# hellosunking/Microcket

Hardware: NVIDIA B200
Metric: valid pairs/sec (SAM->dedup->binned) (higher is better)
Workload: dtype u8

## Files before the change

microcket_b200/csrc/pairs.cu:

```cuda
#include <algorithm>
#include <vector>
#include "mk_common.cuh"
#include "radix_sort.cuh"
#include "pairs_ws.h"

struct K64 {
    typedef u64 Key;
    static constexpr int ITEMS = 16;
    static constexpr int MIN_BLOCKS = 1;
    static constexpr bool HAS_VAL = false;
    struct Bufs { u64 *k[2]; u32 *v[2]; };
    __device__ static __forceinline__ u32 digit(const u64 &k, int byte) { return (u32)(k >> (8 * byte)) & 255u; }
    __device__ static __forceinline__ u64 load_key(const Bufs &b, int which, u64 i) { return b.k[which][i]; }
    __device__ static __forceinline__ void store_key(const Bufs &b, int which, u64 i, const u64 &k) { b.k[which][i] = k; }
};

#define UQ_T 256
#define UQ_ITEMS 8

__global__ void __launch_bounds__(256) k_mark_first(const u64 *k0, const u64 *k1, const u32 *v0, const u32 *v1, const RadixPlan *plan,
                                                    u64 n, u8 *keep, unsigned long long *n_unique) {
    const u64 *k = plan->final_buf ? k1 : k0;
    const u32 *v = plan->final_buf ? v1 : v0;
    u32 local = 0;
    for (u64 i = (u64)blockIdx.x * blockDim.x + threadIdx.x; i < n; i += (u64)gridDim.x * blockDim.x) {
        bool first = i == 0 || k[i] != k[i - 1];
        keep[plan->n_exec ? v[i] : (u32)i] = first ? 1 : 0;
        local += first;
    }
    local = __reduce_add_sync(0xffffffffu, local);
    if ((threadIdx.x & 31) == 0 && local) atomicAdd(n_unique, (unsigned long long)local);
}

__device__ __forceinline__ bool pair_key_differs(const uint4 &a, const uint4 &b) {
    return a.x != b.x || a.y != b.y || a.z != b.z || ((a.w ^ b.w) & 0xFFFF00FFu) != 0;
}

__global__ void __launch_bounds__(UQ_T) k_unique_rec16(const uint4 *b0, const uint4 *b1, const RadixPlan *plan, u64 n,
                                                       uint4 *o0, uint4 *o1, u64 *desc, unsigned long long *n_out, u32 *ticket) {
    __shared__ u32 s_scan[UQ_T / 32 + 1];
    __shared__ u64 s_base;
    __shared__ u32 s_tile;
    const uint4 *in = plan->final_buf ? b1 : b0;
    uint4 *out = plan->final_buf ? o0 : o1;
    const int tid = threadIdx.x, lane = tid & 31, wid = tid >> 5;
    const int n_tiles = (int)((n + UQ_T * UQ_ITEMS - 1) / (UQ_T * UQ_ITEMS));
    while (true) {
        if (tid == 0) s_tile = atomicAdd(ticket, 1u);
        __syncthreads();
        const int tile = (int)s_tile;
        if (tile >= n_tiles) break;
        const u64 base = (u64)tile * UQ_T * UQ_ITEMS + (u64)tid * UQ_ITEMS;
        uint4 r[UQ_ITEMS]; u32 f = 0, cnt = 0;
        uint4 prev = base > 0 && base <= n ? in[base - 1] : make_uint4(0, 0, 0, 0);
#pragma unroll
        for (int k = 0; k < UQ_ITEMS; ++k) {
            if (base + k < n) {
                r[k] = in[base + k];
                bool first = (base + k == 0) || pair_key_differs(r[k], prev);
                prev = r[k];
                if (first) { f |= 1u << k; ++cnt; }
            }
        }
        u32 tot;
        u32 ex = block_excl_scan<UQ_T>(cnt, s_scan, &tot);
        if (wid == 0) {
            u64 b = lookback_exclusive(desc, tile, 0, tot, lane);
            if (lane == 0) { s_base = b; if (tile == n_tiles - 1) *n_out = b + tot; }
        }
        __syncthreads();
        u64 o = s_base + ex;
// ... 44 lines not shown
}

__global__ void k_rle_trim(const u64 *key, const u32 *pos, unsigned long long *counters , u64 n, u64 cap) {
    const u64 runs = counters[0];
    counters[2] = n;
    if (runs && runs <= cap && key[runs - 1] == 0xFFFFFFFFFFFFFFFFull) { counters[0] = runs - 1; counters[2] = pos[runs - 1]; }
}
__global__ void k_rle_finish(const u64 *key, const u32 *pos, const unsigned long long *nnz_p, u64 n_unused, u64 cap,
                             u32 *bin1, u32 *bin2, u32 *cnt) {
    const u64 n = nnz_p[2];
    const u64 nnz = *nnz_p < cap ? *nnz_p : cap;
    for (u64 i = (u64)blockIdx.x * blockDim.x + threadIdx.x; i < nnz; i += (u64)gridDim.x * blockDim.x) {
        u64 k = key[i];
        bin1[i] = (u32)(k >> 32); bin2[i] = (u32)k;
        u32 nxt = (i + 1 < *nnz_p && i + 1 < cap) ? pos[i + 1] : (u32)n;
        if (i + 1 < *nnz_p && i + 1 >= cap) nxt = pos[i] + 1;
        cnt[i] = nxt - pos[i];
    }
}

#define BIN_BAD_KEY 0xFFFFFFFFFFFFFFFFull
__global__ void k_bin_keys(const mk_pair *p, u64 n, const u32 *chr_off , const u32 *chr_len , u32 n_ids,
                           u32 res, u64 *key, unsigned long long *bad) {
    u32 nbad = 0;
    for (u64 i = (u64)blockIdx.x * blockDim.x + threadIdx.x; i < n; i += (u64)gridDim.x * blockDim.x) {
        const uint4 r = ((const uint4 *)p)[i];
        const u32 pos1 = r.x, pos2 = r.y, c1 = r.z & 0xFFFFu, c2 = r.z >> 16;
        u64 k = BIN_BAD_KEY;
        if (c1 < n_ids && c2 < n_ids && pos1 <= chr_len[c1] && pos2 <= chr_len[c2]) {
            u32 a = chr_off[c1] + pos1 / res, b = chr_off[c2] + pos2 / res;
            if (a > b) { u32 t = a; a = b; b = t; }
            k = ((u64)a << 32) | b;
        }
        nbad += k == BIN_BAD_KEY;
        key[i] = k;
    }
    nbad = __reduce_add_sync(0xffffffffu, nbad);
    if ((threadIdx.x & 31) == 0 && nbad) atomicAdd(bad, (unsigned long long)nbad);
}

extern "C" int mk_pairs_ws_create(int device, size_t max_pairs, mk_pairs_ws **out) {
    if (!out || max_pairs == 0) { mk_set_error("mk_pairs_ws_create: bad argument"); return MK_ERR_ARG; }
    int ndev = 0;
    if (cudaGetDeviceCount(&ndev) != cudaSuccess || ndev == 0) { mk_set_error("no CUDA device: microcket_b200 has no CPU fallback"); return MK_ERR_CUDA; }
    MK_CUDA(cudaSetDevice(device));
    mk_pairs_ws *w = new mk_pairs_ws();
    w->device = device; w->sms = mk_sm_count(device); w->max_pairs = max_pairs;
    int rc = w->rws.alloc(max_pairs);
    if (rc == MK_OK) rc = w->alt.alloc(max_pairs * 16);
    if (rc == MK_OK) rc = w->keys2.alloc(max_pairs * 8);
    if (rc == MK_OK) rc = w->heads_key.alloc(max_pairs * 8);
    if (rc == MK_OK) rc = w->heads_pos.alloc(max_pairs * 4);
    if (rc == MK_OK) rc = w->desc.alloc((max_pairs / (UQ_T * UQ_ITEMS) + 4) * 8 + 2048);
    if (rc == MK_OK) rc = w->counter.alloc(64);
    if (rc == MK_OK) rc = w->chr_off.alloc(65536 * 8 + 16384 * 8);
    if (rc == MK_OK && cudaMemset(w->chr_off.p, 0, w->chr_off.n) != cudaSuccess) rc = MK_ERR_CUDA;
    if (rc != MK_OK) { delete w; return rc; }
    *out = w;
    return MK_OK;
}
extern "C" void mk_pairs_ws_destroy(mk_pairs_ws *w) { if (w) { cudaSetDevice(w->device); delete w; } }
extern "C" uint64_t mk_pairs_launch_count(mk_pairs_ws *w) { return w ? w->launches : 0; }
extern "C" uint64_t mk_pairs_dropped(mk_pairs_ws *w) { return w ? w->dropped : 0; }

static int lookback_grid(const void *kernel, int threads, int sms) {
    int occ = 1;
    cudaOccupancyMaxActiveBlocksPerMultiprocessor(&occ, kernel, threads, 0);
    return sms * std::max(1, std::min(occ, 4));
}

extern "C" int mk_pairs_dedup_device(mk_pairs_ws *w, mk_pair *d_pairs, size_t n, size_t *n_kept, void *stream) {
    if (!w || !n_kept) { mk_set_error("mk_pairs_dedup_device: bad argument"); return MK_ERR_ARG; }
    if (n > w->max_pairs) { mk_set_error("mk_pairs_dedup_device: workspace holds %zu pairs, got %zu", w->max_pairs, n); return MK_ERR_CAPACITY; }
    MK_CUDA(cudaSetDevice(w->device));
    cudaStream_t s = (cudaStream_t)stream;
    if (n == 0) { *n_kept = 0; return MK_OK; }
    RadixSchedule sch; sch.n_pass = 15;
    const int order[15] = {12, 4, 5, 6, 7, 10, 11, 0, 1, 2, 3, 8, 9, 14, 15};
    for (int i = 0; i < 15; ++i) sch.byte_of[i] = order[i];
    Rec16::Bufs b; b.k[0] = (uint4 *)d_pairs; b.k[1] = w->alt.as<uint4>(); b.v[0] = b.v[1] = nullptr;
    MK_TRY(radix_sort<Rec16>(b, n, sch, w->rws, 0, w->sms, s, &w->launches));
    const int n_tiles = (int)((n + UQ_T * UQ_ITEMS - 1) / (UQ_T * UQ_ITEMS));
    MK_CUDA(cudaMemsetAsync(w->desc.p, 0, (size_t)(n_tiles + 1) * 8, s));
    MK_CUDA(cudaMemsetAsync(w->counter.p, 0, 64, s));
    k_unique_rec16<<<lookback_grid((const void *)k_unique_rec16, UQ_T, w->sms), UQ_T, 0, s>>>(
        b.k[0], b.k[1], w->rws.plan.as<RadixPlan>(), n, b.k[0], b.k[1], w->desc.as<u64>(), w->counter.as<unsigned long long>(),
        (u32 *)(w->counter.as<unsigned long long>() + 4));
    w->launches += 1;
    struct { unsigned long long kept; } hc;
    u32 final_buf = 0;
    MK_CUDA(cudaMemcpyAsync(&hc, w->counter.p, 8, cudaMemcpyDeviceToHost, s));
    MK_CUDA(cudaMemcpyAsync(&final_buf, (char *)w->rws.plan.p + offsetof(RadixPlan, final_buf), 4, cudaMemcpyDeviceToHost, s));
    MK_CUDA(cudaStreamSynchronize(s));
    if (final_buf == 0) MK_CUDA(cudaMemcpyAsync(d_pairs, w->alt.p, (size_t)hc.kept * 16, cudaMemcpyDeviceToDevice, s));
    *n_kept = (size_t)hc.kept;
    MK_CUDA(cudaStreamSynchronize(s));
    return MK_OK;
}

extern "C" int mk_pairs_bin_device(mk_pairs_ws *w, const mk_pair *d_pairs, size_t n, const uint32_t *chrom_len, int n_chrom,
                                   const uint16_t *chrom_id_map, int n_map, uint32_t res, uint32_t *d_bin1, uint32_t *d_bin2,
                                   uint32_t *d_cnt, size_t cap, size_t *nnz, void *stream) {
    if (!w || !nnz || !chrom_len || n_chrom <= 0 || res == 0) { mk_set_error("mk_pairs_bin_device: bad argument"); return MK_ERR_ARG; }
    if (n > w->max_pairs) { mk_set_error("mk_pairs_bin_device: workspace holds %zu pairs, got %zu", w->max_pairs, n); return MK_ERR_CAPACITY; }
    MK_CUDA(cudaSetDevice(w->device));
    cudaStream_t s = (cudaStream_t)stream;
    if (n == 0) { *nnz = 0; return MK_OK; }
    std::vector<u64> off(n_chrom + 1, 0);
    for (int c = 0; c < n_chrom; ++c) off[c + 1] = off[c] + chrom_len[c] / res + 1;
    if (off[n_chrom] >= (1ull << 32)) { mk_set_error("mk_pairs_bin_device: more than 2^32 bins"); return MK_ERR_CAPACITY; }
    const int n_ids = chrom_id_map ? n_map : n_chrom;
    if (n_ids > 65536) { mk_set_error("mk_pairs_bin_device: too many chromosome ids"); return MK_ERR_ARG; }
    std::vector<u32> by_id(2 * (size_t)n_ids);
    for (int i = 0; i < n_ids; ++i) {
        int c = chrom_id_map ? chrom_id_map[i] : i;
        if (c < 0 || c >= n_chrom) { mk_set_error("mk_pairs_bin_device: chromosome map entry %d out of range", i); return MK_ERR_ARG; }
        by_id[i] = (u32)off[c]; by_id[n_ids + i] = chrom_len[c];
    }
    MK_CUDA(cudaMemcpyAsync(w->chr_off.p, by_id.data(), by_id.size() * 4, cudaMemcpyHostToDevice, s));
    MK_CUDA(cudaMemsetAsync(w->counter.p, 0, 64, s));
// ... 99 lines not shown
        u32 peers = __match_any_sync(0xffffffffu, d);
        if (i < n && lane == __ffs(peers) - 1) atomicAdd(&s_c[d], (u32)__popc(peers));
    }
    __syncthreads();
    if (threadIdx.x < world && s_c[threadIdx.x]) atomicAdd(&counts[threadIdx.x], (unsigned long long)s_c[threadIdx.x]);
}

__global__ void __launch_bounds__(256) k_owner_scatter(const mk_pair *p, u64 n, u32 world, u32 res, unsigned long long *cursor ,
                                                       mk_pair *out) {
    const int lane = threadIdx.x & 31;
    const u64 n_round = (n + 31) & ~(u64)31;
    for (u64 i = (u64)blockIdx.x * blockDim.x + threadIdx.x; i < n_round; i += (u64)gridDim.x * blockDim.x) {
        u32 d = 0xFFFFu + lane; uint4 r = make_uint4(0, 0, 0, 0);
        if (i < n) { r = ((const uint4 *)p)[i]; d = mk_owner_hash(r.z & 0xFFFFu, r.z >> 16, r.x / res) % world; }
        u32 peers = __match_any_sync(0xffffffffu, d);
        int leader = __ffs(peers) - 1;
        unsigned long long base = 0;
        if (i < n && lane == leader) base = atomicAdd(&cursor[d], (unsigned long long)__popc(peers));
        base = __shfl_sync(0xffffffffu, base, leader);
        if (i < n) ((uint4 *)out)[base + __popc(peers & ((1u << lane) - 1u))] = r;
    }
}

__global__ void k_owner_prefix(unsigned long long *dc, u32 world) {
    unsigned long long run = 0;
    for (u32 r = 0; r < world; ++r) { dc[64 + r] = run; run += dc[r]; }
}

extern "C" int mk_pairs_partition_device(mk_pairs_ws *w, const mk_pair *d_pairs, size_t n, int world, uint32_t res, mk_pair *d_out,
                                         uint64_t *counts, void *stream) {
    if (!w || !counts || world < 1 || world > 64 || res == 0 || (n && (!d_pairs || !d_out))) { mk_set_error("mk_pairs_partition_device: bad argument"); return MK_ERR_ARG; }
    if (n > w->max_pairs) { mk_set_error("mk_pairs_partition_device: workspace holds %zu pairs, got %zu", w->max_pairs, n); return MK_ERR_CAPACITY; }
    MK_CUDA(cudaSetDevice(w->device));
    cudaStream_t s = (cudaStream_t)stream;
    unsigned long long *dc = (unsigned long long *)w->desc.p;
    MK_CUDA(cudaMemsetAsync(dc, 0, 128 * 8, s));
    if (n) {
        k_owner_count<<<w->sms * 8, 256, 0, s>>>(d_pairs, n, (u32)world, res, dc);
        k_owner_prefix<<<1, 1, 0, s>>>(dc, (u32)world);
    }
    unsigned long long h[64];
    MK_CUDA(cudaMemcpyAsync(h, dc, (size_t)world * 8, cudaMemcpyDeviceToHost, s));
    if (n) k_owner_scatter<<<w->sms * 8, 256, 0, s>>>(d_pairs, n, (u32)world, res, dc + 64, d_out);
    w->launches += n ? 3 : 0;
    MK_CUDA(cudaStreamSynchronize(s));
    for (int r = 0; r < world; ++r) counts[r] = h[r];
    return MK_OK;
}

extern "C" uint32_t mk_pairs_owner(uint32_t chr1, uint32_t chr2, uint32_t pos1, uint32_t res, uint32_t world) {
    return mk_owner_hash(chr1, chr2, pos1 / res) % world;
}

struct PackCfg { u32 res, nb, nr, nl, total_bits, n_dec, n_ids, max_lane; };

__device__ __forceinline__ void put_bits(u64 &lo, u64 &hi, u64 v, u32 width) {
    hi = width >= 64 ? lo << (width - 64) : (width ? (hi << width) | (lo >> (64 - width)) : hi);
    lo = width >= 64 ? 0 : lo << width;
    lo |= v;
}
__device__ __forceinline__ u64 take_bits(u64 &lo, u64 &hi, u32 width) {
    const u64 v = width >= 64 ? lo : (lo & ((1ull << width) - 1));
    lo = width >= 64 ? hi : (width ? (lo >> width) | (hi << (64 - width)) : lo);
    hi = width >= 64 ? 0 : hi >> width;
    return v;
}

__global__ void __launch_bounds__(256) k_pack_keys(const mk_pair *p, u64 n, const u32 *off_by_id, const u32 *len_by_id, PackCfg c, uint4 *key,
                                                   unsigned long long *bad, RadixSchedule sch, RadixPlan *plan) {
    extern __shared__ u32 s_hist[];
    for (int i = threadIdx.x; i < sch.n_pass * 256; i += 256) s_hist[i] = 0;
    __syncthreads();
    const int lane_id = threadIdx.x & 31;
    u32 nbad = 0;
    const u64 n_round = (n + 31) & ~(u64)31;
    for (u64 i = (u64)blockIdx.x * blockDim.x + threadIdx.x; i < n_round; i += (u64)gridDim.x * blockDim.x) {
        const bool valid = i < n;
        uint4 k = make_uint4(0xFFFFFFFFu, 0xFFFFFFFFu, 0xFFFFFFFFu, (u32)i);
        if (valid) {
            const uint4 r = ((const uint4 *)p)[i];
            u32 pos1 = r.x, pos2 = r.y; const u32 c1 = r.z & 0xFFFFu, c2 = r.z >> 16;
            u32 st = r.w & 3u; const u32 lane = r.w >> 16;
            bool ok = c1 < c.n_ids && c2 < c.n_ids && lane <= c.max_lane;
            if (ok) {
                const u32 q1 = pos1 / c.res, q2 = pos2 / c.res;
                ok = pos1 <= len_by_id[c1] && pos2 <= len_by_id[c2];
                if (ok) {
                    u32 a = off_by_id[c1] + q1, b = off_by_id[c2] + q2;
                    u32 r1 = pos1 - q1 * c.res, r2 = pos2 - q2 * c.res;
                    u32 sw = 0;
                    if (a > b) { u32 t = a; a = b; b = t; t = r1; r1 = r2; r2 = t; st = ((st & 1u) << 1) | (st >> 1); sw = 1; }
                    u64 lo = 0, hi = 0;
                    put_bits(lo, hi, a, c.nb); put_bits(lo, hi, b, c.nb); put_bits(lo, hi, lane, c.nl);
                    put_bits(lo, hi, r1, c.nr); put_bits(lo, hi, r2, c.nr); put_bits(lo, hi, sw, 1); put_bits(lo, hi, st, 2);
                    k.x = (u32)lo; k.y = (u32)(lo >> 32); k.z = (u32)hi;
                }
            }
            nbad += !ok;
            key[i] = k;
        }
        radix_hist_add<Rec16>(s_hist, sch, k, valid, lane_id);
    }
    nbad = __reduce_add_sync(0xffffffffu, nbad);
    if ((threadIdx.x & 31) == 0 && nbad) atomicAdd(bad, (unsigned long long)nbad);
    __syncthreads();
    radix_hist_flush(s_hist, sch.n_pass, plan);
}

__device__ __forceinline__ u32 chrom_of_bin(u32 bin, u32 hint, const PackCfg &c, const u32 *dec_off) {
    if (dec_off[hint] <= bin && (hint + 1 == c.n_dec || bin < dec_off[hint + 1])) return hint;
    u32 l = 0, h = c.n_dec - 1;
    while (l < h) { const u32 m = (l + h + 1) >> 1; if (dec_off[m] <= bin) l = m; else h = m - 1; }
    return l;
}
__device__ __forceinline__ mk_pair unpack_key(uint4 k, const PackCfg &c, const u32 *dec_off, const u16 *dec_id, u32 &hint) {
    u64 lo = (u64)k.x | ((u64)k.y << 32), hi = (u64)k.z;
    u32 st = (u32)take_bits(lo, hi, 2); const u32 sw = (u32)take_bits(lo, hi, 1);
    u32 r2 = (u32)take_bits(lo, hi, c.nr), r1 = (u32)take_bits(lo, hi, c.nr);
    const u32 lane = (u32)take_bits(lo, hi, c.nl);
    u32 b = (u32)take_bits(lo, hi, c.nb), a = (u32)take_bits(lo, hi, c.nb);
    u32 ka = chrom_of_bin(a, hint, c, dec_off);
    u32 kb = chrom_of_bin(b, ka, c, dec_off);
    hint = ka;
    if (sw) { u32 t = a; a = b; b = t; t = r1; r1 = r2; r2 = t; t = ka; ka = kb; kb = t; st = ((st & 1u) << 1) | (st >> 1); }
    mk_pair o;
    o.pos1 = (a - dec_off[ka]) * c.res + r1; o.pos2 = (b - dec_off[kb]) * c.res + r2;
    o.chr1 = dec_id[ka]; o.chr2 = dec_id[kb]; o.strands = (u8)st; o.lane = (u16)lane;
    if (o.chr1 != o.chr2) o.cls = 0;
    else { const u32 d = o.pos2 - o.pos1; o.cls = d >= 10000u ? 1 : (d >= 1000u ? 2 : 3); }
    return o;
}

__global__ void __launch_bounds__(UQ_T) k_uniq_cells(const uint4 *b0, const uint4 *b1, const RadixPlan *plan, u64 n, PackCfg c,
                                                     const u32 *dec_off, const u16 *dec_id, mk_pair *out0, mk_pair *out1,
                                                     u32 *cell_b1, u32 *cell_b2, u32 *cell_first, u64 cell_cap, u8 *keep, u32 *kept_idx,
                                                     u64 *desc, unsigned long long *counters , u32 *ticket) {
    __shared__ u32 s_w[2][UQ_T / 32];
    __shared__ u64 s_base;
    __shared__ u32 s_tile;
    const uint4 *in = plan->final_buf ? b1 : b0;
    mk_pair *out = plan->final_buf ? out0 : out1;
    const int tid = threadIdx.x, lane = tid & 31, wid = tid >> 5;
    const int n_tiles = (int)((n + UQ_T * UQ_ITEMS - 1) / (UQ_T * UQ_ITEMS));
    const u32 cell_shift = c.total_bits - 2 * c.nb;
    while (true) {
        if (tid == 0) s_tile = atomicAdd(ticket, 1u);
        __syncthreads();
        const int tile = (int)s_tile;
        if (tile >= n_tiles) break;
        const u64 base = (u64)tile * UQ_T * UQ_ITEMS + (u64)tid * UQ_ITEMS;
        uint4 r[UQ_ITEMS]; u32 fk = 0, fc = 0, nk = 0, nc = 0;
        uint4 prev = base > 0 && base <= n ? in[base - 1] : make_uint4(0, 0, 0, 0);
#pragma unroll
        for (int k = 0; k < UQ_ITEMS; ++k) {
            if (base + k < n) {
                r[k] = in[base + k];
                const bool first = base + k == 0;
                const bool dk = first || r[k].x != prev.x || r[k].y != prev.y || r[k].z != prev.z;
                bool dc = first;
                if (!first && dk) {
                    u64 lo = (u64)r[k].x | ((u64)r[k].y << 32), hi = (u64)r[k].z;
                    u64 plo = (u64)prev.x | ((u64)prev.y << 32), phi = (u64)prev.z;
                    take_bits(lo, hi, cell_shift); take_bits(plo, phi, cell_shift);
                    dc = lo != plo || hi != phi;
                }
                prev = r[k];
                if (dk) { fk |= 1u << k; ++nk; }
                if (dc) { fc |= 1u << k; ++nc; }
            }
        }
        const u32 ik = warp_incl_scan(nk, lane), ic = warp_incl_scan(nc, lane);
        if (lane == 31) { s_w[0][wid] = ik; s_w[1][wid] = ic; }
        __syncthreads();
        u32 bk = 0, bc = 0, tk = 0, tc = 0;
#pragma unroll
        for (int w = 0; w < UQ_T / 32; ++w) { const u32 x = s_w[0][w], y = s_w[1][w]; tk += x; tc += y; if (w < wid) { bk += x; bc += y; } }
        if (wid == 0) {
            const u64 agg = (u64)tk | ((u64)tc << 31);
            const u64 b = lookback_exclusive(desc, tile, 0, agg, lane);
            if (lane == 0) { s_base = b; if (tile == n_tiles - 1) { counters[0] = (b & 0x7FFFFFFFu) + tk; counters[1] = (b >> 31) + tc; } }
        }
        __syncthreads();
        u64 ok = (s_base & 0x7FFFFFFFu) + bk + ik - nk, oc = (s_base >> 31) + bc + ic - nc;
        u32 hint = 0;
#pragma unroll
        for (int k = 0; k < UQ_ITEMS; ++k) {
            if (fc & (1u << k)) {
                if (oc < cell_cap) {
                    u64 lo = (u64)r[k].x | ((u64)r[k].y << 32), hi = (u64)r[k].z;
                    take_bits(lo, hi, cell_shift);
                    const u32 bb = (u32)take_bits(lo, hi, c.nb), aa = (u32)take_bits(lo, hi, c.nb);
                    cell_b1[oc] = aa; cell_b2[oc] = bb; cell_first[oc] = (u32)ok;
                }
                ++oc;
            }
            if (fk & (1u << k)) {
                out[ok] = unpack_key(r[k], c, dec_off, dec_id, hint);
                if (keep) keep[r[k].w] = 1;
                if (kept_idx) kept_idx[ok] = r[k].w;
                ++ok;
            }
        }
        __syncthreads();
    }
}

__global__ void k_uniq_trim(const uint4 *b0, const uint4 *b1, const RadixPlan *plan, u64 n, u8 *keep, unsigned long long *counters) {
    const uint4 *in = plan->final_buf ? b1 : b0;
    if (!counters[3]) return;
    const u64 first_bad = n - counters[3];
    const uint4 k = in[first_bad];
    if (k.x == 0xFFFFFFFFu && k.y == 0xFFFFFFFFu && k.z == 0xFFFFFFFFu) {
        counters[0] -= 1; counters[1] -= 1;
        if (keep) keep[k.w] = 0;
    }
}

__global__ void k_cell_counts(const u32 *cell_first, const unsigned long long *counters, u64 cap, u32 *cnt) {
    const u64 kept = counters[0], cells = counters[1] < cap ? counters[1] : cap;
    for (u64 i = (u64)blockIdx.x * blockDim.x + threadIdx.x; i < cells; i += (u64)gridDim.x * blockDim.x)
        cnt[i] = (i + 1 < counters[1] && i + 1 < cap ? cell_first[i + 1] : (u32)kept) - cell_first[i];
}

__global__ void k_copy_if_alt(const RadixPlan *plan, u32 keys_in_home_when, const uint4 *alt, uint4 *home, const unsigned long long *counters) {
    if (plan->final_buf != keys_in_home_when) return;
    const u64 n = counters[0];
    for (u64 i = (u64)blockIdx.x * blockDim.x + threadIdx.x; i < n; i += (u64)gridDim.x * blockDim.x) home[i] = alt[i];
}

static u32 bits_for(u64 max_value) { u32 b = 1; while (b < 64 && (max_value >> b)) ++b; return b; }

extern "C" int mk_pairs_dedup_bin_indexed_device(mk_pairs_ws *w, mk_pair *d_pairs, size_t n, const uint32_t *chrom_len, int n_chrom,
                                                 const uint16_t *chrom_id_map, int n_map, uint32_t res, uint16_t max_lane,
                                                 uint32_t *d_bin1, uint32_t *d_bin2, uint32_t *d_cnt, size_t cap,
                                                 uint8_t *d_keep, uint32_t *d_kept_idx, size_t *n_kept, size_t *nnz, void *stream) {
    if (!w || !n_kept || !nnz || !chrom_len || n_chrom <= 0 || res == 0 || !d_bin1 || !d_bin2 || !d_cnt) { mk_set_error("mk_pairs_dedup_bin_device: bad argument"); return MK_ERR_ARG; }
    if (n > w->max_pairs) { mk_set_error("mk_pairs_dedup_bin_device: workspace holds %zu pairs, got %zu", w->max_pairs, n); return MK_ERR_CAPACITY; }
    MK_CUDA(cudaSetDevice(w->device));
    cudaStream_t s = (cudaStream_t)stream;
    *n_kept = 0; *nnz = 0; w->dropped = 0;
    if (n == 0) return MK_OK;
    std::vector<u64> off(n_chrom + 1, 0);
    for (int c = 0; c < n_chrom; ++c) off[c + 1] = off[c] + chrom_len[c] / res + 1;
    if (off[n_chrom] >= (1ull << 32)) { mk_set_error("mk_pairs_dedup_bin_device: more than 2^32 bins"); return MK_ERR_CAPACITY; }
    const int n_ids = chrom_id_map ? n_map : n_chrom;
    if (n_ids > 16384 || n_chrom > 16384) { mk_set_error("mk_pairs_dedup_bin_device: too many chromosomes"); return MK_ERR_ARG; }
    std::vector<u32> tab(3 * 16384 + 8192, 0);
    u32 *by_id = tab.data(), *nb_id = by_id + 16384, *dec_off = nb_id + 16384; u16 *dec_id = (u16 *)(dec_off + 16384);
    for (int c = 0; c < n_chrom; ++c) { dec_off[c] = (u32)off[c]; dec_id[c] = 0xFFFF; }
    for (int i = 0; i < n_ids; ++i) {
        int c = chrom_id_map ? chrom_id_map[i] : i;
        if (c < 0 || c >= n_chrom) { mk_set_error("mk_pairs_dedup_bin_device: chromosome map entry %d out of range", i); return MK_ERR_ARG; }
        by_id[i] = (u32)off[c]; nb_id[i] = chrom_len[c];
        if (dec_id[c] == 0xFFFF) dec_id[c] = (u16)i;
    }
    PackCfg pc; pc.res = res; pc.nb = bits_for(off[n_chrom]) ;
    pc.nr = bits_for(res - 1); pc.nl = max_lane ? bits_for(max_lane) : 0;
    pc.total_bits = 2 * pc.nb + 2 * pc.nr + pc.nl + 3; pc.n_dec = (u32)n_chrom; pc.n_ids = (u32)n_ids; pc.max_lane = max_lane;
    if (pc.total_bits > 96) { mk_set_error("mk_pairs_dedup_bin_device: key needs %u bits, 96 available", pc.total_bits); return MK_ERR_CAPACITY; }
    u32 *d_by_id = w->chr_off.as<u32>(), *d_nb_id = d_by_id + 16384, *d_dec_off = d_nb_id + 16384; u16 *d_dec_id = (u16 *)(d_dec_off + 16384);
    MK_CUDA(cudaMemcpyAsync(d_by_id, tab.data(), tab.size() * 4, cudaMemcpyHostToDevice, s));
    MK_CUDA(cudaMemsetAsync(w->counter.p, 0, 64, s));
    unsigned long long *cnt = w->counter.as<unsigned long long>();
    if (d_keep) MK_CUDA(cudaMemsetAsync(d_keep, 0, n, s));
    RadixSchedule sch; sch.n_pass = (int)((pc.total_bits + 7) / 8);
    for (int i = 0; i < sch.n_pass; ++i) sch.byte_of[i] = i;
    const bool in_place = (sch.n_pass & 1) != 0;
    uint4 *k0 = in_place ? (uint4 *)d_pairs : w->alt.as<uint4>(), *k1 = in_place ? w->alt.as<uint4>() : (uint4 *)d_pairs;
    MK_CUDA(cudaMemsetAsync(w->rws.plan.p, 0, sizeof(RadixPlan), s));
    k_pack_keys<<<w->sms * 8, 256, sch.n_pass * 256 * 4, s>>>(d_pairs, n, d_by_id, d_nb_id, pc, k0, cnt + 3, sch, w->rws.plan.as<RadixPlan>());
    w->launches += 1;
    Rec16::Bufs b; b.k[0] = k0; b.k[1] = k1; b.v[0] = b.v[1] = nullptr;
    MK_TRY(radix_sort<Rec16>(b, n, sch, w->rws, 0, w->sms, s, &w->launches, true));
    const int n_tiles = (int)((n + UQ_T * UQ_ITEMS - 1) / (UQ_T * UQ_ITEMS));
    MK_CUDA(cudaMemsetAsync(w->desc.p, 0, (size_t)(n_tiles + 1) * 8, s));
    const RadixPlan *plan = w->rws.plan.as<RadixPlan>();
    k_uniq_cells<<<lookback_grid((const void *)k_uniq_cells, UQ_T, w->sms), UQ_T, 0, s>>>(
        k0, k1, plan, n, pc, d_dec_off, d_dec_id, (mk_pair *)k0, (mk_pair *)k1,
        d_bin1, d_bin2, w->heads_pos.as<u32>(), cap, d_keep, d_kept_idx, w->desc.as<u64>(), cnt, (u32 *)(cnt + 4));
    k_uniq_trim<<<1, 1, 0, s>>>(k0, k1, plan, n, d_keep, cnt);
    k_cell_counts<<<w->sms * 4, 256, 0, s>>>(w->heads_pos.as<u32>(), cnt, cap, d_cnt);
    k_copy_if_alt<<<w->sms * 4, 256, 0, s>>>(plan, in_place ? 0u : 1u, w->alt.as<uint4>(), (uint4 *)d_pairs, cnt);
    w->launches += 4;
    unsigned long long h[4];
    MK_CUDA(cudaMemcpyAsync(h, cnt, 32, cudaMemcpyDeviceToHost, s));
    MK_CUDA(cudaStreamSynchronize(s));
    *n_kept = (size_t)h[0]; *nnz = (size_t)h[1]; w->dropped = h[3];
    if (h[1] > cap) { mk_set_error("mk_pairs_dedup_bin_device: %llu non-zero cells, output capacity %zu", h[1], cap); return MK_ERR_CAPACITY; }
    return MK_OK;
}

extern "C" int mk_pairs_dedup_bin_device(mk_pairs_ws *w, mk_pair *d_pairs, size_t n, const uint32_t *chrom_len, int n_chrom,
                                         const uint16_t *chrom_id_map, int n_map, uint32_t res, uint16_t max_lane,
                                         uint32_t *d_bin1, uint32_t *d_bin2, uint32_t *d_cnt, size_t cap,
                                         size_t *n_kept, size_t *nnz, void *stream) {
    return mk_pairs_dedup_bin_indexed_device(w, d_pairs, n, chrom_len, n_chrom, chrom_id_map, n_map, res, max_lane, d_bin1, d_bin2, d_cnt, cap,
                                             nullptr, nullptr, n_kept, nnz, stream);
}
```

microcket_b200/csrc/pairs_ws.h:

```cpp
#pragma once
#include "mk_common.cuh"
#include "radix_sort.cuh"

struct mk_pairs_ws {
    int device = 0, sms = 148;
    size_t max_pairs = 0;
    RadixWs rws;
    DevBuf alt;
    DevBuf keys2;
    DevBuf heads_key, heads_pos;
    DevBuf desc, counter, chr_off;
    DevBuf h_pairs, h_b1, h_b2, h_c;
    DevBuf sort2;
    DevBuf tile_sum, tile_off; size_t text_tiles = 0;
    DevBuf names, nl;
    u64 launches = 0;
    u64 dropped = 0;
    int text_scratch(size_t n_tiles) {
        if (n_tiles <= text_tiles) return MK_OK;
        MK_TRY(tile_sum.alloc(n_tiles * 4)); MK_TRY(tile_off.alloc(n_tiles * 8));
        text_tiles = n_tiles;
        return MK_OK;
    }
};
```

Measured before the change: 1.873 billion.

## Stage uniq tile loads and pair outputs through padded shared memory for coalescing

Loads each tile of sorted 16-byte keys into padded shared memory with a coalesced strided pattern, instead of each thread reading eight consecutive records. Unpacked mk_pair outputs are compacted into the same shared buffer and then written to global memory coalesced as uint4. The aim is to replace uncoalesced per-thread global loads and scattered stores with contiguous transactions. In exchange it adds about 66KB of shared memory per block, which may reduce occupancy, plus two extra block barriers, and it relies on mk_pair fitting in 16 bytes.

Measured after the change: 1.889 billion, median of 6. About the same (+0.9%).

```diff
diff --git a/microcket_b200/csrc/pairs.cu b/microcket_b200/csrc/pairs.cu
--- a/microcket_b200/csrc/pairs.cu
+++ b/microcket_b200/csrc/pairs.cu
@@ -465,6 +465,7 @@
     return o;
 }
 
+#define UQ_PAD(i) ((i) + (i) / UQ_ITEMS)
 __global__ void __launch_bounds__(UQ_T) k_uniq_cells(const uint4 *b0, const uint4 *b1, const RadixPlan *plan, u64 n, PackCfg c,
                                                      const u32 *dec_off, const u16 *dec_id, mk_pair *out0, mk_pair *out1,
                                                      u32 *cell_b1, u32 *cell_b2, u32 *cell_first, u64 cell_cap, u8 *keep, u32 *kept_idx,
@@ -472,8 +473,9 @@
     __shared__ u32 s_w[2][UQ_T / 32];
     __shared__ u64 s_base;
     __shared__ u32 s_tile;
+    __shared__ uint4 s_rec[UQ_PAD(UQ_T * UQ_ITEMS)];
     const uint4 *in = plan->final_buf ? b1 : b0;
-    mk_pair *out = plan->final_buf ? out0 : out1;
+    uint4 *out = (uint4 *)(plan->final_buf ? out0 : out1);
     const int tid = threadIdx.x, lane = tid & 31, wid = tid >> 5;
     const int n_tiles = (int)((n + UQ_T * UQ_ITEMS - 1) / (UQ_T * UQ_ITEMS));
     const u32 cell_shift = c.total_bits - 2 * c.nb;
@@ -482,13 +484,20 @@
         __syncthreads();
         const int tile = (int)s_tile;
         if (tile >= n_tiles) break;
-        const u64 base = (u64)tile * UQ_T * UQ_ITEMS + (u64)tid * UQ_ITEMS;
+        const u64 tile_base = (u64)tile * UQ_T * UQ_ITEMS, base = tile_base + (u64)tid * UQ_ITEMS;
+        const u32 n_tile = (u32)min((u64)UQ_T * UQ_ITEMS, n - tile_base);
+#pragma unroll
+        for (int k = 0; k < UQ_ITEMS; ++k) {
+            const u32 i = k * UQ_T + tid;
+            if (i < n_tile) s_rec[UQ_PAD(i)] = in[tile_base + i];
+        }
+        __syncthreads();
         uint4 r[UQ_ITEMS]; u32 fk = 0, fc = 0, nk = 0, nc = 0;
-        uint4 prev = base > 0 && base <= n ? in[base - 1] : make_uint4(0, 0, 0, 0);
+        uint4 prev = base > 0 && base <= n ? (tid ? s_rec[UQ_PAD(tid * UQ_ITEMS - 1)] : in[base - 1]) : make_uint4(0, 0, 0, 0);
 #pragma unroll
         for (int k = 0; k < UQ_ITEMS; ++k) {
             if (base + k < n) {
-                r[k] = in[base + k];
+                r[k] = s_rec[UQ_PAD(tid * UQ_ITEMS + k)];
                 const bool first = base + k == 0;
                 const bool dk = first || r[k].x != prev.x || r[k].y != prev.y || r[k].z != prev.z;
                 bool dc = first;
@@ -515,7 +524,9 @@
             if (lane == 0) { s_base = b; if (tile == n_tiles - 1) { counters[0] = (b & 0x7FFFFFFFu) + tk; counters[1] = (b >> 31) + tc; } }
         }
         __syncthreads();
-        u64 ok = (s_base & 0x7FFFFFFFu) + bk + ik - nk, oc = (s_base >> 31) + bc + ic - nc;
+        const u64 tile_k = s_base & 0x7FFFFFFFu;
+        u32 lk = bk + ik - nk;
+        u64 oc = (s_base >> 31) + bc + ic - nc;
         u32 hint = 0;
 #pragma unroll
         for (int k = 0; k < UQ_ITEMS; ++k) {
@@ -524,17 +535,19 @@
                     u64 lo = (u64)r[k].x | ((u64)r[k].y << 32), hi = (u64)r[k].z;
                     take_bits(lo, hi, cell_shift);
                     const u32 bb = (u32)take_bits(lo, hi, c.nb), aa = (u32)take_bits(lo, hi, c.nb);
-                    cell_b1[oc] = aa; cell_b2[oc] = bb; cell_first[oc] = (u32)ok;
+                    cell_b1[oc] = aa; cell_b2[oc] = bb; cell_first[oc] = (u32)(tile_k + lk);
                 }
                 ++oc;
             }
             if (fk & (1u << k)) {
-                out[ok] = unpack_key(r[k], c, dec_off, dec_id, hint);
+                *(mk_pair *)&s_rec[UQ_PAD(lk)] = unpack_key(r[k], c, dec_off, dec_id, hint);
                 if (keep) keep[r[k].w] = 1;
-                if (kept_idx) kept_idx[ok] = r[k].w;
-                ++ok;
+                if (kept_idx) kept_idx[tile_k + lk] = r[k].w;
+                ++lk;
             }
         }
+        __syncthreads();
+        for (u32 i = tid; i < tk; i += UQ_T) out[tile_k + i] = s_rec[UQ_PAD(i)];
         __syncthreads();
     }
 }
```

## Replace full LSD radix sort with top-byte sort plus in-shared-memory segment sort

Applied to the files above, without the earlier changes.

The dedup/bin path now radix-sorts only the top three key bytes globally. Windows of 2048 records are then finished with an in-shared-memory LSD sort over only the low bytes that actually vary. Prefix groups that overflow a window are gathered, fully sorted by a separate global radix sort, and scattered back. The single lookback unique kernel becomes per-tile count, scan and emit kernels. This cuts global sort passes, at the cost of a host sync mid-pipeline, extra launches, and complex boundary logic.

New measurement: 1.873 billion before, 1.938 billion after, median of 6. 3.5% higher.

```diff
diff --git a/microcket_b200/csrc/pairs.cu b/microcket_b200/csrc/pairs.cu
--- a/microcket_b200/csrc/pairs.cu
+++ b/microcket_b200/csrc/pairs.cu
@@ -17,6 +17,10 @@
 
 #define UQ_T 256
 #define UQ_ITEMS 8
+#define DB_T 2048
+#define DB_THREADS 512
+#define DB_ITEMS 8
+#define DB_WARPS (DB_THREADS / 32)
 
 __global__ void __launch_bounds__(256) k_mark_first(const u64 *k0, const u64 *k1, const u32 *v0, const u32 *v1, const RadixPlan *plan,
                                                     u64 n, u8 *keep, unsigned long long *n_unique) {
@@ -167,6 +171,7 @@
     if (rc == MK_OK) rc = w->heads_key.alloc(max_pairs * 8);
     if (rc == MK_OK) rc = w->heads_pos.alloc(max_pairs * 4);
     if (rc == MK_OK) rc = w->desc.alloc((max_pairs / (UQ_T * UQ_ITEMS) + 4) * 8 + 2048);
+    if (rc == MK_OK) rc = w->seg.alloc((max_pairs / DB_T + 2) * 5 * 4);
     if (rc == MK_OK) rc = w->counter.alloc(64);
     if (rc == MK_OK) rc = w->chr_off.alloc(65536 * 8 + 16384 * 8);
     if (rc == MK_OK && cudaMemset(w->chr_off.p, 0, w->chr_off.n) != cudaSuccess) rc = MK_ERR_CUDA;
@@ -178,9 +183,9 @@
 extern "C" uint64_t mk_pairs_launch_count(mk_pairs_ws *w) { return w ? w->launches : 0; }
 extern "C" uint64_t mk_pairs_dropped(mk_pairs_ws *w) { return w ? w->dropped : 0; }
 
-static int lookback_grid(const void *kernel, int threads, int sms) {
+static int lookback_grid(const void *kernel, int threads, int sms, size_t smem = 0) {
     int occ = 1;
-    cudaOccupancyMaxActiveBlocksPerMultiprocessor(&occ, kernel, threads, 0);
+    cudaOccupancyMaxActiveBlocksPerMultiprocessor(&occ, kernel, threads, smem);
     return sms * std::max(1, std::min(occ, 4));
 }
 
@@ -386,7 +391,7 @@
     return mk_owner_hash(chr1, chr2, pos1 / res) % world;
 }
 
-struct PackCfg { u32 res, nb, nr, nl, total_bits, n_dec, n_ids, max_lane; };
+struct PackCfg { u32 res, nb, nr, nl, total_bits, n_dec, n_ids, max_lane, pshift , pbits ; };
 
 __device__ __forceinline__ void put_bits(u64 &lo, u64 &hi, u64 v, u32 width) {
     hi = width >= 64 ? lo << (width - 64) : (width ? (hi << width) | (lo >> (64 - width)) : hi);
@@ -465,77 +470,234 @@
     return o;
 }
 
-__global__ void __launch_bounds__(UQ_T) k_uniq_cells(const uint4 *b0, const uint4 *b1, const RadixPlan *plan, u64 n, PackCfg c,
-                                                     const u32 *dec_off, const u16 *dec_id, mk_pair *out0, mk_pair *out1,
-                                                     u32 *cell_b1, u32 *cell_b2, u32 *cell_first, u64 cell_cap, u8 *keep, u32 *kept_idx,
-                                                     u64 *desc, unsigned long long *counters , u32 *ticket) {
-    __shared__ u32 s_w[2][UQ_T / 32];
-    __shared__ u64 s_base;
-    __shared__ u32 s_tile;
+__device__ __forceinline__ u32 key_prefix(const uint4 &r, const PackCfg &c) {
+    u64 lo = (u64)r.x | ((u64)r.y << 32), hi = (u64)r.z;
+    take_bits(lo, hi, c.pshift);
+    return (u32)lo & ((1u << c.pbits) - 1u);
+}
+__device__ u64 prefix_bound(const uint4 *in, const PackCfg &c, u64 lo, u64 hi, u32 p, bool upper) {
+    while (lo < hi) {
+        const u64 m = (lo + hi) >> 1;
+        const u32 q = key_prefix(in[m], c);
+        if (q < p || (upper && q == p)) lo = m + 1; else hi = m;
+    }
+    return lo;
+}
+
+__global__ void k_over_find(const uint4 *b0, const uint4 *b1, const RadixPlan *plan, u64 n, PackCfg c, u32 n_win, u32 *seg_start, u32 *seg_len) {
+    const uint4 *in = plan->final_buf ? b1 : b0;
+    for (u32 t = blockIdx.x * blockDim.x + threadIdx.x; t < n_win; t += gridDim.x * blockDim.x) {
+        const u64 a = (u64)t * DB_T, e = a + DB_T < n ? a + DB_T : n;
+        u64 start = 0, len = 0;
+        if (t >= 1) {
+            const u32 p = key_prefix(in[a - 1], c);
+            if (key_prefix(in[e - 1], c) == p && !(t >= 2 && key_prefix(in[a - DB_T - 1], c) == p)) {
+                start = prefix_bound(in, c, 0, a - 1, p, false);
+                len = prefix_bound(in, c, e, n, p, true) - start;
+            }
+        }
+        seg_start[t] = (u32)start; seg_len[t] = (u32)len;
+    }
+}
+
+__global__ void __launch_bounds__(1024) k_scan_windows(const u32 *cnt, u32 n_win, u32 *off, unsigned long long *total) {
+    __shared__ u32 s_scan[1024 / 32 + 1];
+    const u32 per = (n_win + 1023) / 1024, b = threadIdx.x * per, e = b + per < n_win ? b + per : n_win;
+    u32 sum = 0;
+    for (u32 t = b; t < e; ++t) sum += cnt[t];
+    u32 tot;
+    u32 run = block_excl_scan<1024>(sum, s_scan, &tot);
+    for (u32 t = b; t < e; ++t) { off[t] = run; run += cnt[t]; }
+    if (threadIdx.x == 0) { off[n_win] = tot; *total = tot; }
+}
+
+__device__ __forceinline__ u32 over_src(u32 j, const u32 *off, const u32 *seg_start, u32 n_win) {
+    u32 lo = 0, hi = n_win;
+    while (lo < hi) { const u32 m = (lo + hi + 1) >> 1; if (off[m] <= j) lo = m; else hi = m - 1; }
+    return seg_start[lo] + (j - off[lo]);
+}
+__global__ void k_over_gather(const uint4 *data, uint4 *scr, u32 m, const u32 *off, const u32 *seg_start, u32 n_win) {
+    for (u32 j = blockIdx.x * blockDim.x + threadIdx.x; j < m; j += gridDim.x * blockDim.x) scr[j] = data[over_src(j, off, seg_start, n_win)];
+}
+__global__ void k_over_scatter(uint4 *data, const uint4 *s0, const uint4 *s1, const RadixPlan *plan, u32 m, const u32 *off, const u32 *seg_start, u32 n_win) {
+    const uint4 *scr = plan->final_buf ? s1 : s0;
+    for (u32 j = blockIdx.x * blockDim.x + threadIdx.x; j < m; j += gridDim.x * blockDim.x) data[over_src(j, off, seg_start, n_win)] = scr[j];
+}
+
+__device__ __forceinline__ void seg_flags(const uint4 r, const uint4 p, bool first, u32 cell_shift, bool &dk, bool &dc) {
+    dk = first || r.x != p.x || r.y != p.y || r.z != p.z;
+    dc = first;
+    if (!first && dk) {
+        u64 rl = (u64)r.x | ((u64)r.y << 32), rh = (u64)r.z, pl = (u64)p.x | ((u64)p.y << 32), ph = (u64)p.z;
+        take_bits(rl, rh, cell_shift); take_bits(pl, ph, cell_shift);
+        dc = rl != pl || rh != ph;
+    }
+}
+
+struct SegSmem {
+    uint4 rec[2 * DB_T];
+    u32 wc[DB_WARPS * 256];
+    u32 dig[256];
+    u32 scan[DB_WARPS + 1];
+    u32 vary[3];
+    u32 lo, hi, nk, nc;
+};
+
+__device__ __forceinline__ void seg_sort_pass(SegSmem &s, u32 lo, u32 L, u32 byte, int tid, int lane, int wid) {
+    for (int i = tid; i < DB_WARPS * 256; i += DB_THREADS) s.wc[i] = 0;
+    __syncthreads();
+    uint4 r[DB_ITEMS]; u32 rank[DB_ITEMS / 2] = {};
+    u32 *wc = s.wc + wid * 256;
+    const u32 wbase = (u32)wid * 32 * DB_ITEMS;
+#pragma unroll
+    for (int j = 0; j < DB_ITEMS; ++j) {
+        if (wbase + j * 32 >= L) break;
+        const u32 q = wbase + j * 32 + lane;
+        u32 d = 255u;
+        if (q < L) { r[j] = s.rec[lo + q]; d = Rec16::digit(r[j], byte); }
+        u32 peers = 0xffffffffu;
+#pragma unroll
+        for (int bit = 0; bit < 8; ++bit) { const bool on = (d >> bit) & 1u; const u32 bl = __ballot_sync(0xffffffffu, on); peers &= on ? bl : ~bl; }
+        const int leader = __ffs(peers) - 1;
+        u32 old = 0;
+        if (lane == leader) { old = wc[d]; wc[d] = old + (u32)__popc(peers); }
+        old = __shfl_sync(0xffffffffu, old, leader);
+        rank[j / 2] |= (old + (u32)__popc(peers & ((1u << lane) - 1u))) << (16 * (j & 1));
+        __syncwarp();
+    }
+    __syncthreads();
+    u32 cnt = 0;
+    if (tid < 256) {
+#pragma unroll
+        for (int w = 0; w < DB_WARPS; ++w) { const u32 x = s.wc[w * 256 + tid]; s.wc[w * 256 + tid] = cnt; cnt += x; }
+    }
+    u32 tot;
+    const u32 ex = block_excl_scan<DB_THREADS>(cnt, s.scan, &tot);
+    if (tid < 256) s.dig[tid] = ex;
+    __syncthreads();
+#pragma unroll
+    for (int j = 0; j < DB_ITEMS; ++j) {
+        const u32 q = wbase + j * 32 + lane;
+        if (q < L) { const u32 d = Rec16::digit(r[j], byte); s.rec[lo + s.dig[d] + wc[d] + ((rank[j / 2] >> (16 * (j & 1))) & 0xFFFFu)] = r[j]; }
+    }
+    __syncthreads();
+}
+
+__global__ void __launch_bounds__(DB_THREADS, 2) k_seg_sort(uint4 *b0, uint4 *b1, const RadixPlan *plan, u64 n, PackCfg c,
+                                                            u32 *tile_lo, u32 *kept_cnt, u32 *cell_cnt) {
+    extern __shared__ __align__(16) unsigned char s_raw[];
+    SegSmem &s = *(SegSmem *)s_raw;
+    uint4 *in = plan->final_buf ? b1 : b0;
+    const int tid = threadIdx.x, lane = tid & 31, wid = tid >> 5;
+    const u32 n_win = (u32)((n + DB_T - 1) / DB_T), n_pass = (c.pshift + c.pbits) / 8;
+    const u32 cell_shift = c.total_bits - 2 * c.nb;
+    const u32 none = 0xFFFFFFFFu;
+    const u32 tile = blockIdx.x;
+    if (tid == 0) { s.lo = s.hi = none; s.vary[0] = s.vary[1] = s.vary[2] = 0; s.nk = s.nc = 0; }
+    const u64 a = (u64)tile * DB_T;
+    const uint4 prev = tile ? in[a - 1] : make_uint4(0, 0, 0, 0);
+    for (u32 q = tid; q < DB_T; q += DB_THREADS) if (a + q < n) s.rec[q] = in[a + q];
+    __syncthreads();
+    for (u32 q = tid; q < DB_T; q += DB_THREADS)
+        if (a + q < n && (a + q == 0 || key_prefix(s.rec[q], c) != key_prefix(q ? s.rec[q - 1] : prev, c))) { atomicMin(&s.lo, q); break; }
+    __syncthreads();
+    bool cut_hi = false;
+    if (tile + 1 < n_win) {
+        for (u32 q0 = DB_T; q0 < 2 * DB_T; q0 += DB_THREADS) {
+            const u32 q = q0 + tid;
+            if (a + q < n) s.rec[q] = in[a + q];
+            __syncthreads();
+            if (a + q < n && key_prefix(s.rec[q], c) != key_prefix(s.rec[q - 1], c)) atomicMin(&s.hi, q);
+            __syncthreads();
+            if (s.hi != none) break;
+        }
+        cut_hi = s.hi == none;
+    }
+    const u32 lo = s.lo == none ? 0 : s.lo;
+    const u32 hi = tile + 1 < n_win ? (cut_hi ? DB_T : s.hi) : (u32)(n - a);
+    const u32 L = hi - lo;
+    const bool head_lo = lo > 0 || tile == 0 || key_prefix(s.rec[0], c) != key_prefix(prev, c);
+    const bool presorted = (!head_lo || cut_hi) && key_prefix(s.rec[lo], c) == key_prefix(s.rec[hi - 1], c);
+    if (!presorted) {
+        const uint4 f = s.rec[lo];
+        u32 vx = 0, vy = 0, vz = 0;
+#pragma unroll 4
+        for (u32 q = lo + tid; q < hi; q += DB_THREADS) { const uint4 r = s.rec[q]; vx |= r.x ^ f.x; vy |= r.y ^ f.y; vz |= r.z ^ f.z; }
+        vx = __reduce_or_sync(0xffffffffu, vx); vy = __reduce_or_sync(0xffffffffu, vy); vz = __reduce_or_sync(0xffffffffu, vz);
+        if (lane == 0) { if (vx) atomicOr(&s.vary[0], vx); if (vy) atomicOr(&s.vary[1], vy); if (vz) atomicOr(&s.vary[2], vz); }
+    }
+    __syncthreads();
+    bool moved = false;
+#pragma unroll 1
+    for (u32 byte = 0; byte < n_pass; ++byte)
+        if ((s.vary[byte >> 2] >> (8 * (byte & 3))) & 255u) { seg_sort_pass(s, lo, L, byte, tid, lane, wid); moved = true; }
+    const uint4 pred = lo ? s.rec[lo - 1] : prev;
+    u32 nk = 0, nc = 0;
+    for (u32 q = tid; q < L; q += DB_THREADS) {
+        const uint4 r = s.rec[lo + q];
+        if (moved) in[a + lo + q] = r;
+        bool dk, dc;
+        seg_flags(r, q ? s.rec[lo + q - 1] : pred, a + lo + q == 0, cell_shift, dk, dc);
+        nk += dk; nc += dc;
+    }
+    nk = __reduce_add_sync(0xffffffffu, nk); nc = __reduce_add_sync(0xffffffffu, nc);
+    if (lane == 0) { if (nk) atomicAdd(&s.nk, nk); if (nc) atomicAdd(&s.nc, nc); }
+    __syncthreads();
+    if (tid == 0) {
+        tile_lo[tile] = (u32)(a + lo); kept_cnt[tile] = s.nk; cell_cnt[tile] = s.nc;
+        if (tile == n_win - 1) tile_lo[n_win] = (u32)n;
+    }
+}
+
+__global__ void __launch_bounds__(DB_THREADS) k_seg_emit(const uint4 *b0, const uint4 *b1, const RadixPlan *plan, PackCfg c,
+                                                         const u32 *dec_off, const u16 *dec_id, mk_pair *out0, mk_pair *out1,
+                                                         u32 *cell_b1, u32 *cell_b2, u32 *cell_first, u64 cell_cap, u8 *keep, u32 *kept_idx,
+                                                         const u32 *tile_lo, const u32 *kept_off, const u32 *cell_off) {
+    __shared__ u32 s_bk[DB_WARPS][DB_ITEMS], s_bc[DB_WARPS][DB_ITEMS], s_wk[DB_WARPS], s_wc[DB_WARPS];
     const uint4 *in = plan->final_buf ? b1 : b0;
     mk_pair *out = plan->final_buf ? out0 : out1;
     const int tid = threadIdx.x, lane = tid & 31, wid = tid >> 5;
-    const int n_tiles = (int)((n + UQ_T * UQ_ITEMS - 1) / (UQ_T * UQ_ITEMS));
     const u32 cell_shift = c.total_bits - 2 * c.nb;
-    while (true) {
-        if (tid == 0) s_tile = atomicAdd(ticket, 1u);
-        __syncthreads();
-        const int tile = (int)s_tile;
-        if (tile >= n_tiles) break;
-        const u64 base = (u64)tile * UQ_T * UQ_ITEMS + (u64)tid * UQ_ITEMS;
-        uint4 r[UQ_ITEMS]; u32 fk = 0, fc = 0, nk = 0, nc = 0;
-        uint4 prev = base > 0 && base <= n ? in[base - 1] : make_uint4(0, 0, 0, 0);
-#pragma unroll
-        for (int k = 0; k < UQ_ITEMS; ++k) {
-            if (base + k < n) {
-                r[k] = in[base + k];
-                const bool first = base + k == 0;
-                const bool dk = first || r[k].x != prev.x || r[k].y != prev.y || r[k].z != prev.z;
-                bool dc = first;
-                if (!first && dk) {
-                    u64 lo = (u64)r[k].x | ((u64)r[k].y << 32), hi = (u64)r[k].z;
-                    u64 plo = (u64)prev.x | ((u64)prev.y << 32), phi = (u64)prev.z;
-                    take_bits(lo, hi, cell_shift); take_bits(plo, phi, cell_shift);
-                    dc = lo != plo || hi != phi;
-                }
-                prev = r[k];
-                if (dk) { fk |= 1u << k; ++nk; }
-                if (dc) { fc |= 1u << k; ++nc; }
+    const u32 tile = blockIdx.x, b = tile_lo[tile], L = tile_lo[tile + 1] - b;
+    const u32 wbase = (u32)wid * 32 * DB_ITEMS;
+    u32 nk = 0, nc = 0;
+#pragma unroll
+    for (int j = 0; j < DB_ITEMS; ++j) {
+        const u32 q = wbase + j * 32 + lane;
+        bool dk = false, dc = false;
+        if (q < L) seg_flags(in[b + q], b + q ? in[b + q - 1] : make_uint4(0, 0, 0, 0), b + q == 0, cell_shift, dk, dc);
+        const u32 fk = __ballot_sync(0xffffffffu, dk), fc = __ballot_sync(0xffffffffu, dc);
+        if (lane == 0) { s_bk[wid][j] = fk; s_bc[wid][j] = fc; }
+        nk += __popc(fk); nc += __popc(fc);
+    }
+    if (lane == 0) { s_wk[wid] = nk; s_wc[wid] = nc; }
+    __syncthreads();
+    u64 ok = kept_off[tile], oc = cell_off[tile];
+#pragma unroll
+    for (int w = 0; w < DB_WARPS; ++w) if (w < wid) { ok += s_wk[w]; oc += s_wc[w]; }
+    const u32 below = (1u << lane) - 1u;
+    u32 hint = 0;
+#pragma unroll 1
+    for (int j = 0; j < DB_ITEMS; ++j) {
+        const u32 q = wbase + j * 32 + lane, fk = s_bk[wid][j], fc = s_bc[wid][j];
+        if ((fc >> lane) & 1u) {
+            const u64 o = oc + __popc(fc & below);
+            if (o < cell_cap) {
+                const uint4 r = in[b + q];
+                u64 rl = (u64)r.x | ((u64)r.y << 32), rh = (u64)r.z;
+                take_bits(rl, rh, cell_shift);
+                const u32 bb = (u32)take_bits(rl, rh, c.nb), aa = (u32)take_bits(rl, rh, c.nb);
+                cell_b1[o] = aa; cell_b2[o] = bb; cell_first[o] = (u32)(ok + __popc(fk & below));
             }
         }
-        const u32 ik = warp_incl_scan(nk, lane), ic = warp_incl_scan(nc, lane);
-        if (lane == 31) { s_w[0][wid] = ik; s_w[1][wid] = ic; }
-        __syncthreads();
-        u32 bk = 0, bc = 0, tk = 0, tc = 0;
-#pragma unroll
-        for (int w = 0; w < UQ_T / 32; ++w) { const u32 x = s_w[0][w], y = s_w[1][w]; tk += x; tc += y; if (w < wid) { bk += x; bc += y; } }
-        if (wid == 0) {
-            const u64 agg = (u64)tk | ((u64)tc << 31);
-            const u64 b = lookback_exclusive(desc, tile, 0, agg, lane);
-            if (lane == 0) { s_base = b; if (tile == n_tiles - 1) { counters[0] = (b & 0x7FFFFFFFu) + tk; counters[1] = (b >> 31) + tc; } }
-        }
-        __syncthreads();
-        u64 ok = (s_base & 0x7FFFFFFFu) + bk + ik - nk, oc = (s_base >> 31) + bc + ic - nc;
-        u32 hint = 0;
-#pragma unroll
-        for (int k = 0; k < UQ_ITEMS; ++k) {
-            if (fc & (1u << k)) {
-                if (oc < cell_cap) {
-                    u64 lo = (u64)r[k].x | ((u64)r[k].y << 32), hi = (u64)r[k].z;
-                    take_bits(lo, hi, cell_shift);
-                    const u32 bb = (u32)take_bits(lo, hi, c.nb), aa = (u32)take_bits(lo, hi, c.nb);
-                    cell_b1[oc] = aa; cell_b2[oc] = bb; cell_first[oc] = (u32)ok;
-                }
-                ++oc;
-            }
-            if (fk & (1u << k)) {
-                out[ok] = unpack_key(r[k], c, dec_off, dec_id, hint);
-                if (keep) keep[r[k].w] = 1;
-                if (kept_idx) kept_idx[ok] = r[k].w;
-                ++ok;
-            }
-        }
-        __syncthreads();
+        if ((fk >> lane) & 1u) {
+            const u64 o = ok + __popc(fk & below);
+            const uint4 r = in[b + q];
+            out[o] = unpack_key(r, c, dec_off, dec_id, hint);
+            if (keep) keep[r.w] = 1;
+            if (kept_idx) kept_idx[o] = r.w;
+        }
+        oc += __popc(fc); ok += __popc(fk);
     }
 }
 
@@ -597,8 +759,10 @@
     MK_CUDA(cudaMemsetAsync(w->counter.p, 0, 64, s));
     unsigned long long *cnt = w->counter.as<unsigned long long>();
     if (d_keep) MK_CUDA(cudaMemsetAsync(d_keep, 0, n, s));
-    RadixSchedule sch; sch.n_pass = (int)((pc.total_bits + 7) / 8);
-    for (int i = 0; i < sch.n_pass; ++i) sch.byte_of[i] = i;
+    const int n_pass = (int)((pc.total_bits + 7) / 8), n_pre = std::min(3, n_pass);
+    pc.pshift = 8 * (n_pass - n_pre); pc.pbits = 8 * n_pre;
+    RadixSchedule sch; sch.n_pass = n_pre;
+    for (int i = 0; i < n_pre; ++i) sch.byte_of[i] = n_pass - n_pre + i;
     const bool in_place = (sch.n_pass & 1) != 0;
     uint4 *k0 = in_place ? (uint4 *)d_pairs : w->alt.as<uint4>(), *k1 = in_place ? w->alt.as<uint4>() : (uint4 *)d_pairs;
     MK_CUDA(cudaMemsetAsync(w->rws.plan.p, 0, sizeof(RadixPlan), s));
@@ -606,12 +770,39 @@
     w->launches += 1;
     Rec16::Bufs b; b.k[0] = k0; b.k[1] = k1; b.v[0] = b.v[1] = nullptr;
     MK_TRY(radix_sort<Rec16>(b, n, sch, w->rws, 0, w->sms, s, &w->launches, true));
-    const int n_tiles = (int)((n + UQ_T * UQ_ITEMS - 1) / (UQ_T * UQ_ITEMS));
-    MK_CUDA(cudaMemsetAsync(w->desc.p, 0, (size_t)(n_tiles + 1) * 8, s));
     const RadixPlan *plan = w->rws.plan.as<RadixPlan>();
-    k_uniq_cells<<<lookback_grid((const void *)k_uniq_cells, UQ_T, w->sms), UQ_T, 0, s>>>(
-        k0, k1, plan, n, pc, d_dec_off, d_dec_id, (mk_pair *)k0, (mk_pair *)k1,
-        d_bin1, d_bin2, w->heads_pos.as<u32>(), cap, d_keep, d_kept_idx, w->desc.as<u64>(), cnt, (u32 *)(cnt + 4));
+    const u32 n_win = (u32)((n + DB_T - 1) / DB_T);
+    u32 *seg_start = w->seg.as<u32>(), *seg_len = seg_start + n_win + 1, *seg_off = seg_len + n_win + 1;
+    k_over_find<<<(n_win + 255) / 256, 256, 0, s>>>(k0, k1, plan, n, pc, n_win, seg_start, seg_len);
+    k_scan_windows<<<1, 1024, 0, s>>>(seg_len, n_win, seg_off, cnt + 5);
+    w->launches += 2;
+    unsigned long long m = 0;
+    u32 final_buf = 0;
+    MK_CUDA(cudaMemcpyAsync(&m, cnt + 5, 8, cudaMemcpyDeviceToHost, s));
+    MK_CUDA(cudaMemcpyAsync(&final_buf, (char *)w->rws.plan.p + offsetof(RadixPlan, final_buf), 4, cudaMemcpyDeviceToHost, s));
+    MK_CUDA(cudaStreamSynchronize(s));
+    if (m) {
+        if (!w->over.p) MK_TRY(w->over.alloc(w->max_pairs * 16));
+        if (!w->over_rws.plan.p) MK_TRY(w->over_rws.alloc(w->max_pairs));
+        uint4 *data = final_buf ? k1 : k0, *spare = final_buf ? k0 : k1;
+        const int grid = (int)std::min<u64>((m + 255) / 256, (u64)w->sms * 8);
+        k_over_gather<<<grid, 256, 0, s>>>(data, spare, (u32)m, seg_off, seg_start, n_win);
+        RadixSchedule full; full.n_pass = n_pass;
+        for (int i = 0; i < n_pass; ++i) full.byte_of[i] = i;
+        Rec16::Bufs ob; ob.k[0] = spare; ob.k[1] = w->over.as<uint4>(); ob.v[0] = ob.v[1] = nullptr;
+        MK_TRY(radix_sort<Rec16>(ob, m, full, w->over_rws, 0, w->sms, s, &w->launches));
+        k_over_scatter<<<grid, 256, 0, s>>>(data, ob.k[0], ob.k[1], w->over_rws.plan.as<RadixPlan>(), (u32)m, seg_off, seg_start, n_win);
+        w->launches += 2;
+    }
+    u32 *tile_lo = seg_start, *kept_cnt = seg_len, *cell_cnt = seg_off, *kept_off = seg_off + n_win + 1, *cell_off = kept_off + n_win + 1;
+    const size_t smem = sizeof(SegSmem);
+    MK_CUDA(cudaFuncSetAttribute(k_seg_sort, cudaFuncAttributeMaxDynamicSharedMemorySize, (int)smem));
+    k_seg_sort<<<n_win, DB_THREADS, smem, s>>>(k0, k1, plan, n, pc, tile_lo, kept_cnt, cell_cnt);
+    k_scan_windows<<<1, 1024, 0, s>>>(kept_cnt, n_win, kept_off, cnt);
+    k_scan_windows<<<1, 1024, 0, s>>>(cell_cnt, n_win, cell_off, cnt + 1);
+    k_seg_emit<<<n_win, DB_THREADS, 0, s>>>(k0, k1, plan, pc, d_dec_off, d_dec_id, (mk_pair *)k0, (mk_pair *)k1,
+                                            d_bin1, d_bin2, w->heads_pos.as<u32>(), cap, d_keep, d_kept_idx, tile_lo, kept_off, cell_off);
+    w->launches += 4;
     k_uniq_trim<<<1, 1, 0, s>>>(k0, k1, plan, n, d_keep, cnt);
     k_cell_counts<<<w->sms * 4, 256, 0, s>>>(w->heads_pos.as<u32>(), cnt, cap, d_cnt);
     k_copy_if_alt<<<w->sms * 4, 256, 0, s>>>(plan, in_place ? 0u : 1u, w->alt.as<uint4>(), (uint4 *)d_pairs, cnt);
diff --git a/microcket_b200/csrc/pairs_ws.h b/microcket_b200/csrc/pairs_ws.h
--- a/microcket_b200/csrc/pairs_ws.h
+++ b/microcket_b200/csrc/pairs_ws.h
@@ -12,6 +12,8 @@
     DevBuf desc, counter, chr_off;
     DevBuf h_pairs, h_b1, h_b2, h_c;
     DevBuf sort2;
+    DevBuf seg;
+    DevBuf over; RadixWs over_rws;
     DevBuf tile_sum, tile_off; size_t text_tiles = 0;
     DevBuf names, nl;
     u64 launches = 0;
```
